# WhatAShot/Electrocardio-Panorama

Measured on AMD Instinct MI355X. Metric: ECG-samples/sec (train step), higher is better.
Workload: dtype f32 (conv products: fp32 operands split into fp16 hi+lo = 22-23 bits, block-scaled, 3 fp16 matrix products each, fp32 accumulate; fp32-class, not IEEE fp32)

## Files before the change

electrocardio_panorama_amd/_lib.py:

```python
import ctypes as C
import os

import torch

_HERE = os.path.dirname(os.path.abspath(__file__))
LIB_PATH = os.path.join(_HERE, "csrc", "libnefnet_hip.so")

NEF_OK = 0
_ERR = {-1: "NEF_E_SHAPE", -2: "NEF_E_NULL", -3: "NEF_E_WORKSPACE", -4: "NEF_E_UNSUPPORTED"}

p = C.c_void_p
i32 = C.c_int
i64 = C.c_int64
f32 = C.c_float
sz = C.c_size_t


class ConvArgs(C.Structure):
    _fields_ = [
        ("x", p), ("wp", p), ("y", p), ("bias", p), ("in_scale", p), ("res", p), ("gate", p), ("mask", p),
        ("x_bs", i64), ("x_gs", i64), ("y_bs", i64), ("y_gs", i64), ("sc_bs", i64), ("sc_gs", i64),
        ("res_bs", i64), ("res_gs", i64), ("gate_bs", i64), ("gate_gs", i64),
        ("B", i32), ("T", i32), ("G", i32), ("Cin_g", i32), ("Cout_g", i32), ("K", i32),
        ("relu", i32), ("gate_scale", f32), ("drop_scale", f32), ("drop_p", f32), ("rng_seed", C.c_uint64),
# ... 116 lines not shown
                ("out_elems", i64), ("signal_elems", i64), ("Bt", i32), ("N", i32), ("A", i32), ("fill", i32), ("dtype", i32),
                ("reserved0", i32)]


class PackDesc(C.Structure):
    _fields_ = [("w", p), ("wp", p), ("G", i32), ("Cog", i32), ("Cig", i32), ("K", i32), ("transpose_flip", i32),
                ("wino", i32), ("src_mode", i32), ("src_Cr", i32)]


SIGNATURES = {
    "nef_abi_version": (i32, []),
    "nef_debug_spin_us": (i32, [f32, i32, p]),
    "nef_stem_fwd": (i32, [p, p, p, i32, i32, i32, p]),
    "nef_stem_bwd_ws_bytes": (sz, [i32]),
    "nef_stem_bwd_weight": (i32, [p, p, p, p, p, sz, i32, i32, i32, p]),
    "nef_pack_weights": (i32, [C.POINTER(PackDesc), i32, p]),
    "nef_pack_bytes": (sz, [C.POINTER(PackDesc)]),
    "nef_live_extent": (i32, [p, p, i32, i32, i32, p]),
    "nef_conv_fwd": (i32, [C.POINTER(ConvArgs), p]),
    "nef_conv_fwd_live": (i32, [C.POINTER(ConvArgs), p, i32, p]),
    "nef_conv_args_bytes": (sz, []),
    "nef_conv_bwd_weight_ws_bytes": (sz, [C.POINTER(BwwArgs)]),
    "nef_conv_bwd_weight": (i32, [C.POINTER(BwwArgs), p]),
    "nef_conv_bwd_weight_live": (i32, [C.POINTER(BwwArgs), p, i32, p]),
    "nef_bww_args_bytes": (sz, []),
    "nef_h2_tail_census_ws_bytes": (sz, [i32, i32, i32]),
    "nef_h2_tail_census": (i32, [p, i64, i64, i32, i32, i32, i32, p, i64, i64, p, p, i32, i32, p, f32, f32, p, sz, p, p, p, p]),
    "nef_bwd_weight_clamp_ends": (i32, [p, p, i64, i64, p, i32, i32, i32, i32, i32, p]),
    "nef_chan_sum_ws_bytes": (sz, [i32]),
    "nef_chan_sum": (i32, [p, p, p, sz, i32, i32, i32, p]),
    "nef_convt2_fwd": (i32, [p, p, p, p, i32, i32, i32, i32, i32, p]),
    "nef_convt2_bwd_data": (i32, [p, p, p, i32, i32, i32, i32, i32, p]),
    "nef_group_transpose": (i32, [p, p, i32, i32, i32, p]),
    "nef_convt2_interleave": (i32, [p, p, p, i32, i32, i32, p]),
    "nef_convt2_deinterleave": (i32, [p, p, i32, i32, i32, p]),
# ... 183 lines not shown
```

electrocardio_panorama_amd/csrc/conv_h2.hip:

```cpp
#include <hip/hip_runtime.h>
#include <stdint.h>
#include <stdlib.h>

#include "nefnet_hip.h"
#include "nef_common.h"


typedef float f32x16 __attribute__((ext_vector_type(16)));
typedef float f32x4 __attribute__((ext_vector_type(4)));
typedef float f32x2 __attribute__((ext_vector_type(2)));
typedef float f32x4_a4 __attribute__((ext_vector_type(4), aligned(4)));
typedef _Float16 h16x8 __attribute__((ext_vector_type(8)));
typedef _Float16 h16x2 __attribute__((ext_vector_type(2)));
typedef unsigned u32x4 __attribute__((ext_vector_type(4)));
typedef unsigned u32x2 __attribute__((ext_vector_type(2)));

namespace {

constexpr int KC = 16;
constexpr int NTO = 256;
constexpr int PRO_MAX_CIN = 512;

__device__ __forceinline__ void split2(float x0, float x1, unsigned& h, unsigned& l) {
    x0 = __builtin_amdgcn_fmed3f(x0, -65000.f, 65000.f);
// ... 77 lines not shown
            const _Float16 h = (_Float16)v;
            const _Float16 l = (_Float16)(v - (float)h);
            const int64_t frag = ((((int64_t)g * nc16 + ci / 16) * K + kk) * ncot + co / 32) * 2;
            const int fl = (co & 31) + 32 * ((ci & 15) >> 3);
            d.wp[(frag * 64 + fl) * 8 + (ci & 7)] = h;
            d.wp[((frag + 1) * 64 + fl) * 8 + (ci & 7)] = l;
        }
    }
}

#define NEF_H2_TRACK1(V) amax_ = fmaxf(amax_, fabsf(V));
#define NEF_H2_TRACK2(V, W) amax_ = fmaxf(amax_, fmaxf(fabsf(V), fabsf(W)));
constexpr int H2_OCC1 = 3;
template <int K, int PRO, int TM, bool PACK = false>
__global__ __launch_bounds__(256, (TM == 1 && (PRO & 2) == 0) ? H2_OCC1 : 2) void conv_h2_kernel(nef_conv_args a_, int tps_, int n_tiles_, int m_tiles_,
                                                                                                const int32_t* live_, int live_add_) {
    constexpr int MT = 64 * TM;
    constexpr bool UP = (PRO & 2) != 0, AFF = (PRO & 1) != 0;
    constexpr bool PH = (PRO & 4) != 0;
    static_assert(!PH || (!UP && K == 3), "phase-stacked input: K = 3, no upsampling prologue");
    constexpr bool PF = (PRO & 8) != 0;
    static_assert(!PF || (!UP && !PH && K == 3 && TM == 2 && !PACK), "polyphase forward: K = 3, 128-row tile");
    constexpr int NS = UP ? 2 : 1;
    constexpr int PAD = (K - 1) / 2;
    constexpr int XROW = NTO + K - 1;
    constexpr int P4 = (XROW + 3) / 4 + 1;
    constexpr int PLANE = 4 * P4 * 32;
    constexpr int HALF = 4 * P4 * 16;
#define NEF_H2_WADDR(R, W) (((W) >> 1) * HALF + (((R) & 3) * P4 + ((R) >> 2)) * 16 + ((W) & 1) * 8)
#define NEF_H2_RPOS(S) ((((S) & 3) * P4 + ((S) >> 2)) * 16)
    constexpr int NIT = (XROW + 63) / 64;
// ... 613 lines not shown
                    sv[k] = keep + __shfl_xor(send, off, 64);
                }
            }
            const int r = lo >> 1;
            const int ch = g * Cog + cobase + (r & 3) + 8 * (r >> 2);
            const int64_t nslot = (int64_t)tps * 2;
            const int64_t slot = (int64_t)b0 * nslot + (int64_t)(t0 / NTO) * 2 + wn;
            if (inb) slot_out[((int64_t)ch * a.B * nslot + slot) * 2 + (lo & 1)] = sv[0];
        }
    }
    return -1.f;
#undef a
    };
    kargs_t* ap_ = (kargs_t*)__builtin_amdgcn_kernarg_segment_ptr();
    (void)a_;
    const float over_ = tile_pass(ap_, (int)blockIdx.x, (int)threadIdx.x, tps_, n_tiles_, m_tiles_, 0.f, false, live_, live_add_);
    if (over_ > 0.f) {
        int e_;
        (void)frexpf(over_, &e_);
        int bid_ = (int)blockIdx.x, tid_ = (int)threadIdx.x, tps2_ = tps_, nt2_ = n_tiles_, mt2_ = m_tiles_;
        asm volatile("" : "+s"(ap_), "+s"(bid_), "+s"(tps2_), "+s"(nt2_), "+s"(mt2_));
        asm volatile("" : "+v"(tid_));
        (void)tile_pass(ap_, bid_, tid_, tps2_, nt2_, mt2_, ldexpf(1.f, 9 - e_ < 100 ? 9 - e_ : 100), true, nullptr, 0);
    }
}

template <int K, int PRO, int TM, bool PACK = false>
int launch_h2(const nef_conv_args& a, hipStream_t st, const int32_t* live = nullptr, int live_add = 0) {
    constexpr int MT = 64 * TM;
    constexpr int XROW = NTO + K - 1;
    constexpr int P4 = (XROW + 3) / 4 + 1;
    constexpr int PLANE = 4 * P4 * 32;
    constexpr size_t lds = (size_t)4 * PLANE + (((PRO & 1) ? 2 * PRO_MAX_CIN : 0) + 8 * MT + 4) * sizeof(float);
    static unsigned long long lds_set = 0;
    if (int e = nef_ensure_dyn_lds(reinterpret_cast<const void*>(&conv_h2_kernel<K, PRO, TM, PACK>), lds, &lds_set)) return e;
    const int tps = PACK ? (NTO + 4) / (a.T + 4) : (a.T + NTO - 1) / NTO;
    const int n_tiles = PACK ? (a.B + tps - 1) / tps : a.B * tps;
    const int m_tiles = a.Cout_g / MT;
    const int64_t blocks = (int64_t)a.G * m_tiles * n_tiles;
    if (blocks <= 0 || blocks > 0x7fffffff) return NEF_E_SHAPE;
    hipLaunchKernelGGL((conv_h2_kernel<K, PRO, TM, PACK>), dim3((unsigned)blocks), dim3(256), lds, st, a, tps, n_tiles, m_tiles, live, live_add);
    return nef_launch_status();
}

}

static bool h2_pack_shape(const nef_conv_args* a) {
    if (!(a->T >= 8 && a->T <= 64 && a->T % 4 == 0 && (a->K == 1 || a->K == 3))) return false;
    const int64_t spt = (NTO + 4) / (a->T + 4);
    const int64_t lim = 0x7fffffff / 4;
    return a->pro_mode == 0 && !a->in_scale && !a->res_scale && !a->gate_rowscale && !a->stats && !a->bnb_slots && spt * a->x_bs < lim && spt * a->y_bs < lim &&
           (!a->res || spt * a->res_bs < lim) && (!a->gate || spt * a->gate_bs < lim);
}

__attribute__((visibility("hidden"))) bool nef_h2_ok(const nef_conv_args* a) {
    return (a->K == 1 || a->K == 3 || a->K == 7) && a->Cout_g % 64 == 0 && a->Cin_g % KC == 0 && a->T % 2 == 0 &&
           (a->T >= NTO / 2 || h2_pack_shape(a)) &&
           ((a->pro_mode >= 0 && a->pro_mode <= 4) || a->pro_mode == 8 || a->pro_mode == 9) && (a->K == 3 || a->pro_mode == 0) &&
           !(a->pro_mode && a->in_scale) &&
           (!a->res_scale || (a->res && !(a->pro_mode & 8))) &&
           ((!a->gate_rowscale && a->stats_mode == 0) || (a->gate && !(a->pro_mode & 8) && (a->stats_mode == 0 || (a->stats_mode == 1 && a->stats && !a->bnb_slots)))) &&
           (!(a->pro_mode & 8) || (a->Cout_g % 128 == 0 && a->T >= NTO / 2 && !a->res && !a->gate && !a->mask && !a->relu && a->drop_p <= 0.f &&
                                   !a->bnb_slots && (int64_t)a->Cout_g * a->T * 4 < 0x7fffffff)) &&
           (a->pro_mode != 4 || (a->T >= NTO / 2 && (int64_t)a->Cin_g * a->T * 4 < 0x7fffffff)) &&
           (!(a->pro_mode & 1) || a->Cin_g <= PRO_MAX_CIN);
}

__attribute__((visibility("hidden"))) int nef_h2_launch(const nef_conv_args* a, hipStream_t st, const int32_t* live, int live_add) {
    if (!nef_h2_ok(a)) return NEF_E_SHAPE;
    if ((a->pro_mode & 1) && !(a->pro_a && a->pro_b && a->pro_Bp > 0)) return NEF_E_NULL;
    const bool wide = a->Cout_g % 128 == 0;
    if (a->T < NTO / 2)
        return a->K == 1 ? launch_h2<1, 0, 1, true>(*a, st) : launch_h2<3, 0, 1, true>(*a, st);
    if (a->K == 7) return wide ? launch_h2<7, 0, 2>(*a, st, live, live_add) : launch_h2<7, 0, 1>(*a, st, live, live_add);
    if (a->K == 1) return wide ? launch_h2<1, 0, 2>(*a, st, live, live_add) : launch_h2<1, 0, 1>(*a, st, live, live_add);
    switch (a->pro_mode) {
        case 0: return wide ? launch_h2<3, 0, 2>(*a, st, live, live_add) : launch_h2<3, 0, 1>(*a, st, live, live_add);
        case 1: return wide ? launch_h2<3, 1, 2>(*a, st) : launch_h2<3, 1, 1>(*a, st);
        case 2: return launch_h2<3, 2, 1>(*a, st);
        case 4: return wide ? launch_h2<3, 4, 2>(*a, st) : launch_h2<3, 4, 1>(*a, st);
        case 8: return launch_h2<3, 8, 2>(*a, st);
        case 9: return launch_h2<3, 9, 2>(*a, st);
        default: return launch_h2<3, 3, 1>(*a, st);
    }
}

__attribute__((visibility("hidden"))) int nef_h2_pack_status(const nef_pack_desc* dp) {
    const nef_pack_desc& d = *dp;
    const int co_n = d.transpose_flip ? d.Cig : d.Cog, ci_n = d.transpose_flip ? d.Cog : d.Cig;
    if (d.G <= 0 || co_n % 32 != 0 || ci_n % 16 != 0 || (d.K != 1 && d.K != 3 && d.K != 7)) return NEF_E_SHAPE;
    if (d.src_mode != 0 && !(d.src_mode == 1 && d.K == 3 && d.Cog % 2 == 0 && d.src_Cr >= 0 &&
                             (d.src_Cr == 0 || (d.src_Cr % 64 == 0 && d.Cog == 2 * d.src_Cr)))) return NEF_E_SHAPE;
// ... 21 lines not shown
```

electrocardio_panorama_amd/csrc/conv_mfma.hip:

```cpp
#include "nef_common.h"
#include <stdlib.h>

typedef float f32x16 __attribute__((ext_vector_type(16)));
typedef float f32x4 __attribute__((ext_vector_type(4)));
typedef float f32x2 __attribute__((ext_vector_type(2)));

#ifndef NEF_MFMA_PART
#define NEF_MFMA_PART 0
#endif
#define NEF_PART(n) (NEF_MFMA_PART == 0 || NEF_MFMA_PART == (n))

namespace {

constexpr int NT = 128;
constexpr int WT = 64;

template <int K> struct StageK;
template <> struct StageK<7> { static constexpr int KC = 16; };
template <int K, int TM> struct FwdStage {
    static constexpr int KC = ((K == 7 || K == 3) && TM == 2) ? 8 : StageK<K>::KC;
};
template <> struct StageK<3> { static constexpr int KC = 16; };
template <> struct StageK<1> { static constexpr int KC = 64; };

// ... 1920 lines not shown
}

__global__ void chan_sum_final(const double* __restrict__ part, float* __restrict__ out, int C, int nsplit) {
    const int c = blockIdx.x * blockDim.x + threadIdx.x;
    if (c >= C) return;
    double s = 0.0;
    for (int sp = 0; sp < nsplit; ++sp) s += part[(int64_t)sp * C + c];
    out[c] = (float)s;
}

constexpr int CHAN_SUM_SPLIT = 16;

}

__attribute__((visibility("hidden"))) bool nef_h2_ok(const nef_conv_args* a);
__attribute__((visibility("hidden"))) int nef_h2_launch(const nef_conv_args* a, hipStream_t st, const int32_t* live, int live_add);
__attribute__((visibility("hidden"))) int nef_h2_pack(const nef_pack_desc* descs, int n, hipStream_t st);
__attribute__((visibility("hidden"))) int nef_h2_pack_status(const nef_pack_desc* d);

__attribute__((visibility("hidden"))) int nef_mfma_wino4_fwd(const nef_conv_args* a, hipStream_t st);
__attribute__((visibility("hidden"))) int nef_mfma_wino_fwd(const nef_conv_args* a, hipStream_t st);

#if NEF_PART(1)
extern "C" {

int nef_abi_version(void) { return 22; }

static int pack_desc_status(const nef_pack_desc& d) {
    NEF_REQUIRE(d.G > 0 && d.Cog > 0 && d.Cig > 0 && d.K > 0 && d.wino >= 0 && d.wino <= 3 &&
                    (!d.wino || d.K == 3 || d.K == 7 || (d.wino == 3 && d.K == 1)), NEF_E_SHAPE);
    NEF_REQUIRE(d.src_mode == 0 || d.wino == 3, NEF_E_UNSUPPORTED);
// ... 43 lines not shown
        for (int i = 0; i < m; ++i) {
            const int64_t e = (int64_t)t.d[i].G * t.d[i].Cog * t.d[i].Cig * (t.d[i].wino ? 1 : t.d[i].K);
            if (e > biggest) biggest = e;
        }
        int gx = (int)nef_cdiv(biggest, 256);
        if (n_f32 == 1) gx = nef_stream_grid(biggest, 256);
        else if (gx > 64) gx = 64;
        hipLaunchKernelGGL(pack_weights_multi_kernel, dim3((unsigned)gx, (unsigned)m), dim3(256), 0, (hipStream_t)stream, t);
    }
    return nef_launch_status();
}

size_t nef_conv_args_bytes(void) { return sizeof(nef_conv_args); }


static int conv_fwd_entry(const nef_conv_args* a, const int32_t* live, int32_t live_add, nef_stream_t stream) {
    NEF_REQUIRE(a && a->x && a->wp && a->y, NEF_E_NULL);
    NEF_REQUIRE(a->B > 0 && a->T > 0 && a->G > 0, NEF_E_SHAPE);
    const int K = a->K;
    NEF_REQUIRE(K == 1 || K == 3 || K == 7, NEF_E_SHAPE);
    NEF_REQUIRE(a->Cout_g % 64 == 0 && a->Cin_g > 0, NEF_E_SHAPE);
    hipStream_t st = (hipStream_t)stream;
    NEF_REQUIRE((!a->stats && !a->bnb_slots) || a->wino == 2 || a->wino == 3, NEF_E_UNSUPPORTED);
    NEF_REQUIRE(!(a->stats && a->bnb_slots), NEF_E_UNSUPPORTED);
    NEF_REQUIRE(!a->bnb_slots || (a->bnb_x && a->bnb_mean && a->bnb_invstd && a->bnb_a && a->bnb_b), NEF_E_NULL);
    NEF_REQUIRE(!a->bnb_slots || a->bnb_Bp > 0, NEF_E_SHAPE);
    NEF_REQUIRE(!a->bnb_slots || !a->bnb_up || a->T % 4 == 0, NEF_E_SHAPE);
    NEF_REQUIRE((!a->res_scale && !a->gate_rowscale && a->stats_mode == 0) || a->wino == 3, NEF_E_UNSUPPORTED);
    if (a->wino == 3) {
        NEF_REQUIRE(nef_h2_ok(a), NEF_E_SHAPE);
        return nef_h2_launch(a, st, live, live_add);
    }
    bool big = (a->Cout_g % 128 == 0);
    if (big) {
        const ColTiling ct0 = make_tiling(a->B, a->T, NT);
        if ((int64_t)a->G * (a->Cout_g / 128) * ct0.n_tiles < 384) big = false;
    }
    const int KC = K == 1 ? FwdStage<1, 1>::KC : (big ? FwdStage<3, 2>::KC : FwdStage<3, 1>::KC);
    static_assert(FwdStage<7, 2>::KC == FwdStage<3, 2>::KC && FwdStage<7, 1>::KC == FwdStage<3, 1>::KC, "stage sizes");
    NEF_REQUIRE(a->Cin_g % KC == 0, NEF_E_SHAPE);
    if (a->wino == 2) return nef_mfma_wino4_fwd(a, st);
    if (a->wino) return nef_mfma_wino_fwd(a, st);
    if (a->pro_mode != 0) {
        NEF_REQUIRE(K == 3 && a->pro_mode >= 1 && a->pro_mode <= 3 && !a->in_scale, NEF_E_UNSUPPORTED);
        NEF_REQUIRE(!(a->pro_mode & 1) || (a->pro_a && a->pro_b && a->pro_Bp > 0), NEF_E_NULL);
        NEF_REQUIRE(!(a->pro_mode & 2) || (a->T % 2 == 0), NEF_E_SHAPE);
// ... 4 lines not shown
        switch (a->pro_mode) {
            case 1: return big ? launch_conv_fwd<3, 2, 1>(*a, st) : launch_conv_fwd<3, 1, 1>(*a, st);
            case 2: return big ? launch_conv_fwd<3, 2, 2>(*a, st) : launch_conv_fwd<3, 1, 2>(*a, st);
            default: return big ? launch_conv_fwd<3, 2, 3>(*a, st) : launch_conv_fwd<3, 1, 3>(*a, st);
        }
    }
    switch (K) {
        case 7: return big ? launch_conv_fwd<7, 2>(*a, st) : launch_conv_fwd<7, 1>(*a, st);
        case 3: return big ? launch_conv_fwd<3, 2>(*a, st) : launch_conv_fwd<3, 1>(*a, st);
        default: return big ? launch_conv_fwd<1, 2>(*a, st) : launch_conv_fwd<1, 1>(*a, st);
    }
}

int nef_conv_fwd(const nef_conv_args* a, nef_stream_t stream) {
    NEF_ENTER();
    return conv_fwd_entry(a, nullptr, 0, stream);
}

int nef_conv_fwd_live(const nef_conv_args* a, const int32_t* live, int32_t live_add, nef_stream_t stream) {
    NEF_ENTER();
    NEF_REQUIRE(live, NEF_E_NULL);
    return conv_fwd_entry(a, live, live_add, stream);
}

int nef_conv_stats_slots(int T, int Cout_g) {
    if (T <= 0 || T % 2 != 0 || Cout_g <= 0 || Cout_g % 64 != 0) return 0;
    const bool wide = (Cout_g % 128 == 0);
    if (T < (wide ? 128 : 256)) return 0;
    const int nto = wide ? 128 : 256;
    return ((T + nto - 1) / nto) * (nto / 128);
}

size_t nef_bww_args_bytes(void) { return sizeof(nef_bww_args); }

size_t nef_conv_bwd_weight_ws_bytes(const nef_bww_args* a) {
    if (!a) return 0;
    const int B = a->B, T = a->T, G = a->G, Cin_g = a->Cin_g, Cout_g = a->Cout_g, K = a->K;
// ... 190 lines not shown
```

electrocardio_panorama_amd/csrc/stem.hip:

```cpp
#include "nef_common.h"

namespace {

constexpr int KW = 15;
constexpr int TP = 64;
constexpr int CPL = 128;

__device__ __forceinline__ void load_window(__amdgpu_buffer_rsrc_t xrow, int L, int tp, float (&xw)[19]) {
    const int base = 4 * tp - 9;
#pragma unroll
    for (int i = 0; i < 19; ++i) {
        const int p = base + i;
        xw[i] = nef_buf_f32(xrow, (p >= 0 && p < L) ? (unsigned)(p * 4) : NEF_OOB, 0);
    }
}

constexpr int FWD_TP = TP - 1;

__global__ __launch_bounds__(256) void stem_fwd_kernel(const float* __restrict__ x, const float* __restrict__ w,
                                                       float* __restrict__ y, int B, int V, int L, int T,
                                                       int tiles_per_row) {
    __shared__ float wl[CPL * 16];
    int bid = blockIdx.x;
    const int tile = bid % tiles_per_row;
// ... 125 lines not shown
    for (int c = 0; c < BW_CPW; ++c)
#pragma unroll
        for (int k = 0; k < KW; ++k) {
            const float s = nef_wave_sum(acc[c][k]);
            if (lane == 0) part[((int64_t)split * V * CPL + ch0 + c) * KW + k] = s;
        }
}

constexpr int MB_SPLIT = 256;
constexpr int MB_HALO = 16;
constexpr int MB_TAIL = 96;
typedef float f32x4s __attribute__((ext_vector_type(4)));

__global__ __launch_bounds__(256) void stem_bwd_weight_mfma_kernel(const float* __restrict__ x, const float* __restrict__ w,
                                                                   const float* __restrict__ gy, float* __restrict__ part,
                                                                   int B, int V, int L, int T) {
    extern __shared__ float xs[];
    const int v = blockIdx.x % V, slot = blockIdx.x / V;
    const int lane = threadIdx.x & 63, wave = __builtin_amdgcn_readfirstlane((int)(threadIdx.x >> 6));
    const int n16 = lane & 15, kk = lane >> 4;
    const int Lc = L / 2;
    const int xlen = MB_HALO + L + MB_TAIL;
    float wb[2][4];
#pragma unroll
    for (int ct = 0; ct < 2; ++ct)
#pragma unroll
        for (int s = 0; s < 4; ++s) {
            const int tap = 4 * s + kk;
            wb[ct][s] = tap < KW ? w[(v * CPL + 32 * wave + 16 * ct + n16) * KW + tap] : 0.f;
        }
    f32x4s acc[2];
#pragma unroll
    for (int ct = 0; ct < 2; ++ct) acc[ct] = f32x4s{0.f, 0.f, 0.f, 0.f};
    for (int b = slot; b < B; b += MB_SPLIT) {
        __syncthreads();
        const float* xrow = x + ((int64_t)b * V + v) * L;
        for (int i = threadIdx.x; i < xlen; i += 256) {
            const int p = i - MB_HALO;
            xs[i] = (p >= 0 && p < L) ? xrow[p] : 0.f;
        }
        __syncthreads();
        const __amdgpu_buffer_rsrc_t grs = nef_rsrc(gy + ((int64_t)b * V * CPL + v * CPL + 32 * wave) * T);
#define NEF_STEM_GLOAD(TP0, DST)                                                                                       \
    _Pragma("unroll") for (int ct_ = 0; ct_ < 2; ++ct_) {                                                           \
        const int tpl_ = (TP0) + 4 * kk;                                                                            \
        DST[ct_] = nef_buf_f32x4(grs, tpl_ + 3 < T ? (unsigned)((n16 * T + tpl_) * 4) : NEF_OOB, (unsigned)(16 * ct_ * T * 4)); \
        if (tpl_ + 3 >= T && tpl_ < T) {                                                                            \
            _Pragma("unroll") for (int r_ = 0; r_ < 4; ++r_)                                                        \
                DST[ct_][r_] = nef_buf_f32(grs, tpl_ + r_ < T ? (unsigned)((n16 * T + tpl_ + r_) * 4) : NEF_OOB,    \
                                           (unsigned)(16 * ct_ * T * 4));                                           \
        }                                                                                                           \
    }
        f32x4s gnext[2];
        NEF_STEM_GLOAD(0, gnext)
        for (int tp0 = 0; tp0 < T; tp0 += 16) {
            f32x4s gcur[2] = {gnext[0], gnext[1]};
            if (tp0 + 16 < T) NEF_STEM_GLOAD(tp0 + 16, gnext)
            const float* p1 = xs + MB_HALO + 4 * (tp0 + n16) - 9 + kk;
            const float* p2 = xs + MB_HALO + 4 * (tp0 + 4 * kk) - 9 + n16;
            float a1[9], a2[9];
#pragma unroll
            for (int o = 0; o < 9; ++o) {
                a1[o] = p1[2 * o];
                a2[o] = p2[2 * o];
            }
#pragma unroll
            for (int ct = 0; ct < 2; ++ct) {
                const int tpl = tp0 + 4 * kk;
                const f32x4s g4 = gcur[ct];
                f32x4s c[3];
#pragma unroll
                for (int i = 0; i < 3; ++i) {
// ... 108 lines not shown
}

int nef_stem_fwd(const float* x, const float* w, float* y, int B, int V, int L, nef_stream_t stream) {
    NEF_ENTER();
    NEF_REQUIRE(x && w && y, NEF_E_NULL);
    NEF_REQUIRE(B > 0 && V > 0 && L >= 4 && L % 4 == 0, NEF_E_SHAPE);
    const int T = L / 4;
    const int tiles = (T + FWD_TP - 1) / FWD_TP;
    hipLaunchKernelGGL(stem_fwd_kernel, dim3((unsigned)((int64_t)B * V * tiles)), dim3(256), 0, (hipStream_t)stream, x,
                       w, y, B, V, L, T, tiles);
    return nef_launch_status();
}

size_t nef_stem_bwd_ws_bytes(int V) { return (size_t)(MB_SPLIT > BW_SPLIT ? MB_SPLIT : BW_SPLIT) * V * CPL * KW * sizeof(float); }

int nef_stem_bwd_weight(const float* x, const float* w, const float* gy, float* gw, void* ws, size_t ws_bytes, int B,
                        int V, int L, nef_stream_t stream) {
    NEF_ENTER();
    NEF_REQUIRE(x && w && gy && gw && ws, NEF_E_NULL);
    NEF_REQUIRE(B > 0 && V > 0 && L >= 4 && L % 4 == 0, NEF_E_SHAPE);
    NEF_REQUIRE(ws_bytes >= nef_stem_bwd_ws_bytes(V), NEF_E_WORKSPACE);
    const int T = L / 4;
    hipStream_t st = (hipStream_t)stream;
    const int n = V * CPL * KW;
    const size_t lds = (size_t)(MB_HALO + L + MB_TAIL) * sizeof(float);
    if (T % 2 == 0 && lds <= 64 * 1024) {
        const int slots = B < MB_SPLIT ? B : MB_SPLIT;
        hipLaunchKernelGGL(stem_bwd_weight_mfma_kernel, dim3((unsigned)(slots * V)), dim3(256), lds, st, x, w, gy, (float*)ws, B,
                           V, L, T);
        hipLaunchKernelGGL(stem_bwd_weight_reduce, dim3((n + 63) / 64), dim3(256), 0, st, (const float*)ws, gw, n, slots);
        return nef_launch_status();
    }
    const int tiles = (T + BW_TP - 1) / BW_TP;
    hipLaunchKernelGGL(stem_bwd_weight_kernel, dim3((unsigned)(BW_SPLIT * V * (CPL / BW_CPB))), dim3(256), 0, st, x, w,
                       gy, (float*)ws, B, V, L, T, tiles);
    hipLaunchKernelGGL(stem_bwd_weight_reduce, dim3((n + 63) / 64), dim3(256), 0, st, (const float*)ws, gw, n, BW_SPLIT);
    return nef_launch_status();
}

}
```

electrocardio_panorama_amd/engine.py:

```python
import os

import torch
from . import _env

from . import ops
from .ops import GV

N_SEG, ROI_BINS = 7, 16
DROP_P = 0.2
BN_EPS, BN_MOM = 1e-5, 0.1


DROPOUT_SITES = ("W_encoder.layer1.0", "W_encoder.layer1.1", "W_encoder.layer1.2", "w_conv.0", "z1_conv.0",
                 "z2_conv1.0", "z2_conv2.0", "z2_conv2.2")


class DropCfg:

    def __init__(self, training, p=DROP_P, masks=None, seed=0, seed_dev=None):
        self.seed_dev = seed_dev
        self.on = bool(training) and p > 0.0
        self.p = p if self.on else 0.0
        self.scale = 1.0 / (1.0 - p) if self.on else 1.0
        self.masks = masks
# ... 25 lines not shown


def block_fwd(xv, P, prefix, K, Cog, drop, in_scale=None, live=None):
    G = xv.G
    h = ops.conv(xv, ops.pack_weight(P[prefix + ".conv1.weight"], G, T=xv.T), Cog, K, relu=True, in_scale=in_scale, live=live,
                 **drop.args(prefix))
    res_conv = (K == 3 and Cog != xv.Cg)
    assert in_scale is None or not res_conv
    if res_conv:
        r = ops.conv(xv, ops.pack_weight(P[prefix + ".residual_conv.weight"], G, T=xv.T), Cog, 1,
                     bias=P[prefix + ".residual_conv.bias"], live=live)
        resv = GV.dense(r, G)
    else:
        resv = xv
    y = ops.conv(GV.dense(h, G), ops.pack_weight(P[prefix + ".conv2.weight"], G, T=xv.T), Cog, K, res=resv, relu=True,
                 res_scale=in_scale, live=_live_add(live, (K - 1) // 2))
    return y, (xv, h, y, prefix, K, Cog, res_conv, drop.scale, in_scale, live)


def block_scale_ok(P, prefix, G, T):
    return all(ops._pack_shape(P[prefix + n], G, False, T, plain=False)[3] == 3 for n in (".conv1.weight", ".conv2.weight")) and T >= 128


def _bwd_f4(K):
    return K in (3, 7)


def _block_pack_requests(P, prefix, G, T, flip):
    w1 = P[prefix + ".conv1.weight"]
    f4 = bool(flip) and _bwd_f4(w1.shape[2])
    reqs = [ops.PackReq(w1, G, flip, T, f4=f4), ops.PackReq(P[prefix + ".conv2.weight"], G, flip, T, f4=f4)]
# ... 52 lines not shown

def _side(device, work=None):
    mode = _env.get("NEF_SIDE_STREAM", "auto")
    if mode == "0" or (mode == "auto" and work is not None and work < _SIDE_MIN_WORK
                       and not torch.cuda.is_current_stream_capturing()):
        return ops._Inline()
    return ops.SideStream.get(device)


def block_bwd(saved, gy, P, grads, out=None, side=None, pre_gated=False, gate_input=False, scale_bwd=False, g2_chan_sum=None):
    xv, h, y, prefix, K, Cog, res_conv, dscale = saved[:8]
    in_scale = saved[8] if len(saved) > 8 else None
    live_x = saved[9] if len(saved) > 9 else None
    live_h = _live_add(live_x, (K - 1) // 2)
    live_y = block_live_out(saved)
    side = side or ops._Inline()
    G, Cig = xv.G, xv.Cg
    g2 = gy if pre_gated else ops.gate(gy, y)
    g2v, hv = GV.dense(g2, G), GV.dense(h, G)
    grads[prefix + ".conv2.weight"] = side.run(lambda: ops.conv_bwd_weight(hv, g2v, K, site=P[prefix + ".conv2.weight"].data_ptr(), live=live_y), h, g2)
    gc1 = ops.conv(g2v, ops.pack_weight(P[prefix + ".conv2.weight"], G, flip=True, T=xv.T, f4=_bwd_f4(K)), Cog, K, gate=hv,
                   gate_scale=dscale, role="conv_bwd_data", live=live_y)
    gc1v = GV.dense(gc1, G)
    grads[prefix + ".conv1.weight"] = side.run(lambda: ops.conv_bwd_weight(xv, gc1v, K, in_scale=in_scale, site=P[prefix + ".conv1.weight"].data_ptr(), live=live_h), xv.t, gc1)
    if res_conv:
        grads[prefix + ".residual_conv.weight"] = side.run(lambda: ops.conv_bwd_weight(xv, g2v, 1, site=P[prefix + ".residual_conv.weight"].data_ptr()), xv.t, g2)
        grads[prefix + ".residual_conv.bias"] = g2_chan_sum if g2_chan_sum is not None else side.run(lambda: ops.chan_sum(g2), g2)
        gres = ops.conv(g2v, ops.pack_weight(P[prefix + ".residual_conv.weight"], G, flip=True, T=xv.T), Cig, 1,
                        role="conv_bwd_data")
        resv = GV.dense(gres, G)
    else:
        resv = g2v
    wp1f = ops.pack_weight(P[prefix + ".conv1.weight"], G, flip=True, T=xv.T, f4=_bwd_f4(K))
    if in_scale is not None and scale_bwd and int(getattr(wp1f, "nef_wino", 0)) == 3 and out is None:
        slots = ops.conv_stats_buffer(wp1f, xv.B, G, Cig, xv.T, xv.t.device)
        if slots is not None:
            gx = ops.conv(gc1v, wp1f, Cig, K, res=resv, gate=xv, gate_scale=1.0, gate_rowscale=in_scale, stats=slots, stats_mode=1,
                          role="conv_bwd_data", live=live_h)
            return gx, ops.slots_to_rows(slots, xv.B)
    return ops.conv(gc1v, wp1f, Cig, K, res=resv,
                    out=out, gate=xv if gate_input else None, gate_scale=1.0, role="conv_bwd_data", live=live_h)


_DEC = (("decoder.1", "0", "1", 128), ("decoder.1", "3", "4", 128), ("decoder.3", "0", "1", 64),
        ("decoder.3", "3", "4", 64))


_HALVES = "decoder.1.double_conv.0.weight#halves"


def _regroup_halves(w, P=None):
    if P is not None:
        hit = P.get(_HALVES)
        if hit is not None and hit[1] is w and hit[2] == w._version:
            return hit[0]
    wg = ops.regroup_halves(w)
# ... 185 lines not shown
            g = ops.conv(gcv, wpf, x.shape[1], 3, role="conv_bwd_data", bnb=bnb)
        g_is_up = bool(up_after and li > 0 and c.shape[2] % 8 == 0 and c.shape[2] >= 16)
        if up_after and li > 0 and not g_is_up:
            g = ops.upsample2_bwd(g)
    return g, bool(saved[0][7]) and not poly_first, shared_B is not None


def _latents(P, x, in_theta, rois, drop, save, pack_side=None):
    B, V, L = x.shape
    T = L // 4
    sv = {}
    r0 = (T - 1) // 2
    win = (r0 - 2, 6) if (T % 2 == 0 and r0 - 2 >= 0 and r0 + 4 <= T) else None
    ops.pack_many(_latent_pack_requests(P, V, T, win, False))
    live = (ops.live_extent(x), 0) if ops.LIVE else None
    a = ops.stem_fwd(x, P["W_encoder.conv1.weight"])
    if pack_side is not None:
        pack_side.join()
    sv["blk_enc"] = []
    for i in range(3):
        a, s = block_fwd(GV.dense(a, V), P, f"W_encoder.layer1.{i}", 7, 128, drop, live=live)
        sv["blk_enc"].append(s)
        live = block_live_out(s)
    e = ops.theta_mlp_fwd(in_theta, P["mlp1.weight"], P["mlp1.bias"])
    if block_scale_ok(P, "w_conv.0", V, T):
        enc, sv["blk_w_conv"] = block_fwd(GV.dense(a, V), P, "w_conv.0", 3, 128, drop, in_scale=(e, V * 128, 128), live=live)
    else:
        ew = ops.chscale_fwd(a, e)
        enc, sv["blk_w_conv"] = block_fwd(GV.dense(ew, V), P, "w_conv.0", 3, 128, drop, live=live)
    live = block_live_out(sv["blk_w_conv"])
# ... 355 lines not shown
    gew = block_bwd(sv["blk_w_conv"], genc, P, grads, side=side, pre_gated=True, scale_bwd=True)
    if isinstance(gew, tuple):
        g, ge = gew
    else:
        g, ge = ops.chscale_bwd(gew, sv["w"], sv["e"], relu_x=True)
    gW1, gb1 = side.run(lambda: ops.theta_mlp_bwd(sv["in_theta"], ge, 128), ge)
    grads["mlp1.weight"], grads["mlp1.bias"] = gW1, gb1
    if early:
        if EARLY_HOOK is not None:
            EARLY_HOOK(P, grads, side)
        else:
            from . import parallel
            parallel.early_reduce(P, grads, getattr(side, "stream", None))
    for i in (2, 1, 0):
        g = block_bwd(sv["blk_enc"][i], g, P, grads, side=side, pre_gated=True, gate_input=(i > 0))
    grads["W_encoder.conv1.weight"] = ops.stem_bwd_weight(sv["x"], P["W_encoder.conv1.weight"], g)


def backward(P, sv, g_outs):
    grads = {}
    side = _side(sv["z1"].device, sv["z1"].numel())
    if "views" in sv:
        gz1, gz2r, gz2b, gz1_sum = _views_bwd(P, sv, g_outs, grads, side)
    else:
        gz1, gz2r, gz2b, gz1_sum = _head_bwd(P, sv, g_outs, grads, side, relu_z1=True)
    _latents_bwd(P, sv, gz1, gz2r, grads, side, z1_pre_gated=True, early=True, gz2b=gz2b, gz1_sum=gz1_sum)
    side.join()
    return grads


def backward2(P, sv, g_outs):
# ... 24 lines not shown
```

electrocardio_panorama_amd/ops.py:

```python
import ctypes as C
import contextlib
import itertools
import os
from typing import NamedTuple, Optional

import torch
from . import _env

from . import _lib

N_SEG, ROI_BINS = 7, 16


def _p(t):
    return None if t is None else t.data_ptr()


def _stream():
    return torch.cuda.current_stream().cuda_stream


def _chk(t, dtype=torch.float32):
    assert t.is_cuda and t.dtype == dtype and t.is_contiguous(), (t.device, t.dtype, t.is_contiguous())
    return t
# ... 152 lines not shown
        _LIVE_ACC_OF[0] = PROFILE
    acc = _LIVE_ACC.setdefault(tag, [0.0, 0])
    acc[0] += frac
    acc[1] += 1
    EXEC_FP16[tag] = 3.0 * acc[0] / acc[1]


def _live_frac(live, pad, T, tile=256):
    if _LIVE_HOST[0] is not live[0]:
        _LIVE_HOST[0], _LIVE_HOST[1] = live[0], live[0].to("cpu", torch.int64)
    tps = (T + tile - 1) // tile
    bound = _LIVE_HOST[1] + int(live[1]) + pad
    return float(((bound + tile - 1) // tile).clamp(0, tps).double().mean()) / tps


def stem_bwd_weight(x, w, gy):
    L = _lib.load()
    _chk(x), _chk(w), _chk(gy)
    B, V, Ln = x.shape
    gw = torch.empty_like(w)
    n = L.nef_stem_bwd_ws_bytes(V)
    ws = workspace(n, x.device)
    ev = _hbm("stem_bwd_weight", x, gy)
    _lib.check(L.nef_stem_bwd_weight(_p(x), _p(w), _p(gy), _p(gw), _p(ws), n, B, V, Ln, _stream()), "nef_stem_bwd_weight")
    _done(ev)
    return gw


_WV = _env.get("NEF_WINOGRAD", "4")
WINOGRAD = _WV != "0"
WINO_FWD = 1 if _WV in ("1", "2") else 2
WINO_BW4 = _WV not in ("1", "2")
WINO_BW7 = _WV not in ("1", "2")


H2 = _env.get("NEF_H2", "1") == "1"


BATCH_HINT = None
# ... 390 lines not shown
                                         _p(invstd), _p(a), _p(b), _p(ws), n, P, N // P, Ct, Ln, eps, momentum, _p(nbt), _stream()),
               "nef_bn_stats_from_slots")
    return mean, invstd, a, b


def _operand(a, xv, in_scale, pro):
    a.x, a.x_bs, a.x_gs = xv.ptr, xv.bs, xv.gs
    if in_scale is not None:
        a.in_scale, a.sc_bs, a.sc_gs = _p(in_scale[0]), in_scale[1], in_scale[2]
    if pro is not None and pro[0]:
        a.pro_mode, a.pro_a, a.pro_b, a.pro_Bp = pro[0], _p(pro[1]), _p(pro[2]), pro[3]


def conv(xv, wp, Cog, K, out=None, bias=None, in_scale=None, res=None, gate=None, gate_scale=1.0, relu=False,
         mask=None, drop_p=0.0, drop_scale=1.0, seed=0, role="conv_fwd", pro=None, seed_dev=None, stats=None, bnb=None,
         x_scale=0.0, tag_extra="", res_scale=None, gate_rowscale=None, stats_mode=0, live=None):
    L = _lib.load()
    if live is not None and not LIVE:
        live = None

    def launch():
        if live is not None:
            _lib.check(L.nef_conv_fwd_live(C.byref(a), _p(live[0]), int(live[1]), _stream()), "nef_conv_fwd_live")
        else:
            _lib.check(L.nef_conv_fwd(C.byref(a), _stream()), "nef_conv_fwd")
    T_out = xv.T * 2 if (pro is not None and pro[0] & 2) else xv.T
    if out is None:
        y = torch.empty(xv.B, xv.G * Cog, T_out, device=xv.t.device, dtype=torch.float32)
        out = GV.dense(y, xv.G)
    a = _lib.ConvArgs()
    _operand(a, xv, in_scale, pro)
    a.wp, a.y, a.y_bs, a.y_gs = _p(wp), out.ptr, out.bs, out.gs
    a.bias = _p(bias)
    a.res = res.ptr if res is not None else None
    a.gate = gate.ptr if gate is not None else None
    a.mask = _p(mask)
    if res is not None:
# ... 1755 lines not shown
```

include/nefnet_hip.h:

```cpp
#ifndef NEFNET_HIP_H
#define NEFNET_HIP_H

#include <stddef.h>
#include <stdint.h>

#ifdef __cplusplus
extern "C" {
#endif

#define NEF_OK 0
#define NEF_E_SHAPE (-1)
#define NEF_E_NULL (-2)
#define NEF_E_WORKSPACE (-3)
#define NEF_E_UNSUPPORTED (-4)

#define NEF_N_SEG 7
#define NEF_ROI_BINS 16

typedef void* nef_stream_t;

int nef_abi_version(void);

int nef_debug_spin_us(float us, int wgs, nef_stream_t stream);

int nef_stem_fwd(const float* x, const float* w, float* y, int B, int V, int L, nef_stream_t stream);
int nef_live_extent(const float* x, int32_t* live, int B, int V, int L, nef_stream_t stream);
size_t nef_stem_bwd_ws_bytes(int V);
int nef_stem_bwd_weight(const float* x, const float* w, const float* gy, float* gw, void* ws, size_t ws_bytes,
                        int B, int V, int L, nef_stream_t stream);

typedef struct nef_pack_desc {
    const float* w;
    float* wp;
    int32_t G, Cog, Cig, K, transpose_flip, wino;
    int32_t src_mode, src_Cr;
} nef_pack_desc;
size_t nef_pack_bytes(const nef_pack_desc* d);
int nef_pack_weights(const nef_pack_desc* descs, int n, nef_stream_t stream);

typedef struct nef_conv_args {
    const float* x;
    const float* wp;
    float* y;
    const float* bias;
// ... 26 lines not shown
    float x_scale;
    int32_t reserved0;
    const float* x_amax;
    float* x_amax_next;
    int32_t* x_clamped;
    const float* res_scale;
    int64_t rs_bs, rs_gs;
    const float* gate_rowscale;
    int64_t gr_bs, gr_gs;
    int32_t stats_mode;
    int32_t reserved1;
} nef_conv_args;

int nef_conv_fwd(const nef_conv_args* a, nef_stream_t stream);
int nef_conv_fwd_live(const nef_conv_args* a, const int32_t* live, int32_t live_add, nef_stream_t stream);
size_t nef_conv_args_bytes(void);

typedef struct nef_bww_args {
    const float* x;
    const float* gy;
    float* gw;
    void* ws;
    const float* in_scale;
    const float* pro_a;
    const float* pro_b;
    const float* x_amax;
    const float* gy_amax;
    float* x_amax_next;
    float* gy_amax_next;
    int32_t* clamped;
// ... 556 lines not shown
```

Before: 9816.

## Zero-fill dead conv tiles early and clip stem weight-grad to live extent

In the h2 conv kernel, tiles lying fully beyond the per-sample live extent (and beyond the residual's live extent when a residual is added) now write zeros directly and exit, skipping the MFMA work. This applies only when there is no bias, stats or BN slots. A new residual-aware live entry point carries the residual's extent through the encoder block forward and backward-data calls. The stem backward-weight kernel also receives the live extent and stops its time loop at the live end rounded up to 16, which assumes gradients and inputs past that point contribute nothing.

Result: faster. 10070, median of 6 (+2.6%).

```diff
diff --git a/electrocardio_panorama_amd/_lib.py b/electrocardio_panorama_amd/_lib.py
--- a/electrocardio_panorama_amd/_lib.py
+++ b/electrocardio_panorama_amd/_lib.py
@@ -154,11 +154,13 @@
     "nef_stem_fwd": (i32, [p, p, p, i32, i32, i32, p]),
     "nef_stem_bwd_ws_bytes": (sz, [i32]),
     "nef_stem_bwd_weight": (i32, [p, p, p, p, p, sz, i32, i32, i32, p]),
+    "nef_stem_bwd_weight_live": (i32, [p, p, p, p, p, sz, i32, i32, i32, p, p]),
     "nef_pack_weights": (i32, [C.POINTER(PackDesc), i32, p]),
     "nef_pack_bytes": (sz, [C.POINTER(PackDesc)]),
     "nef_live_extent": (i32, [p, p, i32, i32, i32, p]),
     "nef_conv_fwd": (i32, [C.POINTER(ConvArgs), p]),
     "nef_conv_fwd_live": (i32, [C.POINTER(ConvArgs), p, i32, p]),
+    "nef_conv_fwd_live_res": (i32, [C.POINTER(ConvArgs), p, i32, i32, p]),
     "nef_conv_args_bytes": (sz, []),
     "nef_conv_bwd_weight_ws_bytes": (sz, [C.POINTER(BwwArgs)]),
     "nef_conv_bwd_weight": (i32, [C.POINTER(BwwArgs), p]),
diff --git a/electrocardio_panorama_amd/csrc/conv_h2.hip b/electrocardio_panorama_amd/csrc/conv_h2.hip
--- a/electrocardio_panorama_amd/csrc/conv_h2.hip
+++ b/electrocardio_panorama_amd/csrc/conv_h2.hip
@@ -115,7 +115,7 @@
 constexpr int H2_OCC1 = 3;
 template <int K, int PRO, int TM, bool PACK = false>
 __global__ __launch_bounds__(256, (TM == 1 && (PRO & 2) == 0) ? H2_OCC1 : 2) void conv_h2_kernel(nef_conv_args a_, int tps_, int n_tiles_, int m_tiles_,
-                                                                                                const int32_t* live_, int live_add_) {
+                                                                                                const int32_t* live_, int live_add_, int zf_, int res_add_) {
     constexpr int MT = 64 * TM;
     constexpr bool UP = (PRO & 2) != 0, AFF = (PRO & 1) != 0;
     constexpr bool PH = (PRO & 4) != 0;
@@ -759,6 +759,37 @@
     };
     kargs_t* ap_ = (kargs_t*)__builtin_amdgcn_kernarg_segment_ptr();
     (void)a_;
+    if constexpr (PRO == 0 && !PACK) {
+        if (zf_) {
+            const int tile = (int)blockIdx.x % n_tiles_, gm = (int)blockIdx.x / n_tiles_;
+            const int mt = gm % m_tiles_, g = gm / m_tiles_;
+            const int full = (n_tiles_ / (8 * tps_)) * (8 * tps_);
+            int b0, t0;
+            if (tile < full) {
+                const int grp = tile / (8 * tps_), r = tile % (8 * tps_);
+                b0 = grp * 8 + (r & 7);
+                t0 = (r >> 3) * NTO;
+            } else {
+                b0 = tile / tps_;
+                t0 = (tile - b0 * tps_) * NTO;
+            }
+            const int e = live_[b0 * ap_->G + g];
+            const bool dead = t0 - PAD >= e + live_add_;
+            if (dead && (zf_ == 1 || t0 >= e + res_add_)) {
+                const int T = ap_->T;
+                const int t = t0 + 4 * ((int)threadIdx.x & 63);
+                float* const yp = ap_->y + (int64_t)b0 * ap_->y_bs + (int64_t)g * ap_->y_gs + (int64_t)(mt * MT) * T + t;
+                if (t + 3 < T) {
+#pragma unroll 8
+                    for (int r = (int)threadIdx.x >> 6; r < MT; r += 4) *reinterpret_cast<f32x4_a4*>(yp + (int64_t)r * T) = f32x4_a4{0.f, 0.f, 0.f, 0.f};
+                } else if (t < T) {
+#pragma unroll 8
+                    for (int r = (int)threadIdx.x >> 6; r < MT; r += 4) *reinterpret_cast<f32x2*>(yp + (int64_t)r * T) = f32x2{0.f, 0.f};
+                }
+                return;
+            }
+        }
+    }
     const float over_ = tile_pass(ap_, (int)blockIdx.x, (int)threadIdx.x, tps_, n_tiles_, m_tiles_, 0.f, false, live_, live_add_);
     if (over_ > 0.f) {
         int e_;
@@ -771,7 +802,7 @@
 }
 
 template <int K, int PRO, int TM, bool PACK = false>
-int launch_h2(const nef_conv_args& a, hipStream_t st, const int32_t* live = nullptr, int live_add = 0) {
+int launch_h2(const nef_conv_args& a, hipStream_t st, const int32_t* live = nullptr, int live_add = 0, const int* res_add = nullptr) {
     constexpr int MT = 64 * TM;
     constexpr int XROW = NTO + K - 1;
     constexpr int P4 = (XROW + 3) / 4 + 1;
@@ -784,7 +815,10 @@
     const int m_tiles = a.Cout_g / MT;
     const int64_t blocks = (int64_t)a.G * m_tiles * n_tiles;
     if (blocks <= 0 || blocks > 0x7fffffff) return NEF_E_SHAPE;
-    hipLaunchKernelGGL((conv_h2_kernel<K, PRO, TM, PACK>), dim3((unsigned)blocks), dim3(256), lds, st, a, tps, n_tiles, m_tiles, live, live_add);
+    int zf = 0;
+    if (PRO == 0 && !PACK && live && !a.bias && !a.stats && !a.bnb_slots) zf = !a.res ? 1 : (res_add ? 2 : 0);
+    hipLaunchKernelGGL((conv_h2_kernel<K, PRO, TM, PACK>), dim3((unsigned)blocks), dim3(256), lds, st, a, tps, n_tiles, m_tiles, live, live_add, zf,
+                       res_add ? *res_add : 0);
     return nef_launch_status();
 }
 
@@ -811,16 +845,16 @@
            (!(a->pro_mode & 1) || a->Cin_g <= PRO_MAX_CIN);
 }
 
-__attribute__((visibility("hidden"))) int nef_h2_launch(const nef_conv_args* a, hipStream_t st, const int32_t* live, int live_add) {
+__attribute__((visibility("hidden"))) int nef_h2_launch(const nef_conv_args* a, hipStream_t st, const int32_t* live, int live_add, const int* res_add) {
     if (!nef_h2_ok(a)) return NEF_E_SHAPE;
     if ((a->pro_mode & 1) && !(a->pro_a && a->pro_b && a->pro_Bp > 0)) return NEF_E_NULL;
     const bool wide = a->Cout_g % 128 == 0;
     if (a->T < NTO / 2)
         return a->K == 1 ? launch_h2<1, 0, 1, true>(*a, st) : launch_h2<3, 0, 1, true>(*a, st);
-    if (a->K == 7) return wide ? launch_h2<7, 0, 2>(*a, st, live, live_add) : launch_h2<7, 0, 1>(*a, st, live, live_add);
-    if (a->K == 1) return wide ? launch_h2<1, 0, 2>(*a, st, live, live_add) : launch_h2<1, 0, 1>(*a, st, live, live_add);
+    if (a->K == 7) return wide ? launch_h2<7, 0, 2>(*a, st, live, live_add, res_add) : launch_h2<7, 0, 1>(*a, st, live, live_add, res_add);
+    if (a->K == 1) return wide ? launch_h2<1, 0, 2>(*a, st, live, live_add, res_add) : launch_h2<1, 0, 1>(*a, st, live, live_add, res_add);
     switch (a->pro_mode) {
-        case 0: return wide ? launch_h2<3, 0, 2>(*a, st, live, live_add) : launch_h2<3, 0, 1>(*a, st, live, live_add);
+        case 0: return wide ? launch_h2<3, 0, 2>(*a, st, live, live_add, res_add) : launch_h2<3, 0, 1>(*a, st, live, live_add, res_add);
         case 1: return wide ? launch_h2<3, 1, 2>(*a, st) : launch_h2<3, 1, 1>(*a, st);
         case 2: return launch_h2<3, 2, 1>(*a, st);
         case 4: return wide ? launch_h2<3, 4, 2>(*a, st) : launch_h2<3, 4, 1>(*a, st);
diff --git a/electrocardio_panorama_amd/csrc/conv_mfma.hip b/electrocardio_panorama_amd/csrc/conv_mfma.hip
--- a/electrocardio_panorama_amd/csrc/conv_mfma.hip
+++ b/electrocardio_panorama_amd/csrc/conv_mfma.hip
@@ -1958,7 +1958,7 @@
 }
 
 __attribute__((visibility("hidden"))) bool nef_h2_ok(const nef_conv_args* a);
-__attribute__((visibility("hidden"))) int nef_h2_launch(const nef_conv_args* a, hipStream_t st, const int32_t* live, int live_add);
+__attribute__((visibility("hidden"))) int nef_h2_launch(const nef_conv_args* a, hipStream_t st, const int32_t* live, int live_add, const int* res_add);
 __attribute__((visibility("hidden"))) int nef_h2_pack(const nef_pack_desc* descs, int n, hipStream_t st);
 __attribute__((visibility("hidden"))) int nef_h2_pack_status(const nef_pack_desc* d);
 
@@ -2032,7 +2032,7 @@
 size_t nef_conv_args_bytes(void) { return sizeof(nef_conv_args); }
 
 
-static int conv_fwd_entry(const nef_conv_args* a, const int32_t* live, int32_t live_add, nef_stream_t stream) {
+static int conv_fwd_entry(const nef_conv_args* a, const int32_t* live, int32_t live_add, const int32_t* res_add, nef_stream_t stream) {
     NEF_REQUIRE(a && a->x && a->wp && a->y, NEF_E_NULL);
     NEF_REQUIRE(a->B > 0 && a->T > 0 && a->G > 0, NEF_E_SHAPE);
     const int K = a->K;
@@ -2047,7 +2047,7 @@
     NEF_REQUIRE((!a->res_scale && !a->gate_rowscale && a->stats_mode == 0) || a->wino == 3, NEF_E_UNSUPPORTED);
     if (a->wino == 3) {
         NEF_REQUIRE(nef_h2_ok(a), NEF_E_SHAPE);
-        return nef_h2_launch(a, st, live, live_add);
+        return nef_h2_launch(a, st, live, live_add, res_add);
     }
     bool big = (a->Cout_g % 128 == 0);
     if (big) {
@@ -2082,13 +2082,19 @@
 
 int nef_conv_fwd(const nef_conv_args* a, nef_stream_t stream) {
     NEF_ENTER();
-    return conv_fwd_entry(a, nullptr, 0, stream);
+    return conv_fwd_entry(a, nullptr, 0, nullptr, stream);
 }
 
 int nef_conv_fwd_live(const nef_conv_args* a, const int32_t* live, int32_t live_add, nef_stream_t stream) {
     NEF_ENTER();
     NEF_REQUIRE(live, NEF_E_NULL);
-    return conv_fwd_entry(a, live, live_add, stream);
+    return conv_fwd_entry(a, live, live_add, nullptr, stream);
+}
+
+int nef_conv_fwd_live_res(const nef_conv_args* a, const int32_t* live, int32_t live_add, int32_t res_add, nef_stream_t stream) {
+    NEF_ENTER();
+    NEF_REQUIRE(live && a && a->res, NEF_E_NULL);
+    return conv_fwd_entry(a, live, live_add, &res_add, stream);
 }
 
 int nef_conv_stats_slots(int T, int Cout_g) {
diff --git a/electrocardio_panorama_amd/csrc/stem.hip b/electrocardio_panorama_amd/csrc/stem.hip
--- a/electrocardio_panorama_amd/csrc/stem.hip
+++ b/electrocardio_panorama_amd/csrc/stem.hip
@@ -163,13 +163,13 @@
 
 __global__ __launch_bounds__(256) void stem_bwd_weight_mfma_kernel(const float* __restrict__ x, const float* __restrict__ w,
                                                                    const float* __restrict__ gy, float* __restrict__ part,
-                                                                   int B, int V, int L, int T) {
+                                                                   int B, int V, int L, int T, const int32_t* __restrict__ live) {
     extern __shared__ float xs[];
     const int v = blockIdx.x % V, slot = blockIdx.x / V;
     const int lane = threadIdx.x & 63, wave = __builtin_amdgcn_readfirstlane((int)(threadIdx.x >> 6));
     const int n16 = lane & 15, kk = lane >> 4;
     const int Lc = L / 2;
-    const int xlen = MB_HALO + L + MB_TAIL;
+    const int xlen_full = MB_HALO + L + MB_TAIL;
     float wb[2][4];
 #pragma unroll
     for (int ct = 0; ct < 2; ++ct)
@@ -183,6 +183,12 @@
     for (int ct = 0; ct < 2; ++ct) acc[ct] = f32x4s{0.f, 0.f, 0.f, 0.f};
     for (int b = slot; b < B; b += MB_SPLIT) {
         __syncthreads();
+        int Tb = T, xlen = xlen_full;
+        if (live) {
+            const int e = live[b * V + v];
+            const int e16 = (e + 15) & ~15;
+            if (e16 < T) Tb = e16 > 0 ? e16 : 0, xlen = MB_HALO + 4 * Tb + 8;
+        }
         const float* xrow = x + ((int64_t)b * V + v) * L;
         for (int i = threadIdx.x; i < xlen; i += 256) {
             const int p = i - MB_HALO;
@@ -202,9 +208,9 @@
     }
         f32x4s gnext[2];
         NEF_STEM_GLOAD(0, gnext)
-        for (int tp0 = 0; tp0 < T; tp0 += 16) {
+        for (int tp0 = 0; tp0 < Tb; tp0 += 16) {
             f32x4s gcur[2] = {gnext[0], gnext[1]};
-            if (tp0 + 16 < T) NEF_STEM_GLOAD(tp0 + 16, gnext)
+            if (tp0 + 16 < Tb) NEF_STEM_GLOAD(tp0 + 16, gnext)
             const float* p1 = xs + MB_HALO + 4 * (tp0 + n16) - 9 + kk;
             const float* p2 = xs + MB_HALO + 4 * (tp0 + 4 * kk) - 9 + n16;
             float a1[9], a2[9];
@@ -343,9 +349,8 @@
 
 size_t nef_stem_bwd_ws_bytes(int V) { return (size_t)(MB_SPLIT > BW_SPLIT ? MB_SPLIT : BW_SPLIT) * V * CPL * KW * sizeof(float); }
 
-int nef_stem_bwd_weight(const float* x, const float* w, const float* gy, float* gw, void* ws, size_t ws_bytes, int B,
-                        int V, int L, nef_stream_t stream) {
-    NEF_ENTER();
+static int stem_bwd_weight_entry(const float* x, const float* w, const float* gy, float* gw, void* ws, size_t ws_bytes, int B,
+                                 int V, int L, const int32_t* live, nef_stream_t stream) {
     NEF_REQUIRE(x && w && gy && gw && ws, NEF_E_NULL);
     NEF_REQUIRE(B > 0 && V > 0 && L >= 4 && L % 4 == 0, NEF_E_SHAPE);
     NEF_REQUIRE(ws_bytes >= nef_stem_bwd_ws_bytes(V), NEF_E_WORKSPACE);
@@ -356,7 +361,7 @@
     if (T % 2 == 0 && lds <= 64 * 1024) {
         const int slots = B < MB_SPLIT ? B : MB_SPLIT;
         hipLaunchKernelGGL(stem_bwd_weight_mfma_kernel, dim3((unsigned)(slots * V)), dim3(256), lds, st, x, w, gy, (float*)ws, B,
-                           V, L, T);
+                           V, L, T, live);
         hipLaunchKernelGGL(stem_bwd_weight_reduce, dim3((n + 63) / 64), dim3(256), 0, st, (const float*)ws, gw, n, slots);
         return nef_launch_status();
     }
@@ -367,4 +372,17 @@
     return nef_launch_status();
 }
 
-}
+int nef_stem_bwd_weight(const float* x, const float* w, const float* gy, float* gw, void* ws, size_t ws_bytes, int B,
+                        int V, int L, nef_stream_t stream) {
+    NEF_ENTER();
+    return stem_bwd_weight_entry(x, w, gy, gw, ws, ws_bytes, B, V, L, nullptr, stream);
+}
+
+int nef_stem_bwd_weight_live(const float* x, const float* w, const float* gy, float* gw, void* ws, size_t ws_bytes, int B,
+                             int V, int L, const int32_t* live, nef_stream_t stream) {
+    NEF_ENTER();
+    NEF_REQUIRE(live, NEF_E_NULL);
+    return stem_bwd_weight_entry(x, w, gy, gw, ws, ws_bytes, B, V, L, live, stream);
+}
+
+}
diff --git a/electrocardio_panorama_amd/engine.py b/electrocardio_panorama_amd/engine.py
--- a/electrocardio_panorama_amd/engine.py
+++ b/electrocardio_panorama_amd/engine.py
@@ -63,7 +63,7 @@
     else:
         resv = xv
     y = ops.conv(GV.dense(h, G), ops.pack_weight(P[prefix + ".conv2.weight"], G, T=xv.T), Cog, K, res=resv, relu=True,
-                 res_scale=in_scale, live=_live_add(live, (K - 1) // 2))
+                 res_scale=in_scale, live=_live_add(live, (K - 1) // 2), res_live=None if (res_conv or live is None) else live[1])
     return y, (xv, h, y, prefix, K, Cog, res_conv, drop.scale, in_scale, live)
 
 
@@ -146,6 +146,7 @@
     live_x = saved[9] if len(saved) > 9 else None
     live_h = _live_add(live_x, (K - 1) // 2)
     live_y = block_live_out(saved)
+    res_live = None if (res_conv or live_y is None) else live_y[1]
     side = side or ops._Inline()
     G, Cig = xv.G, xv.Cg
     g2 = gy if pre_gated else ops.gate(gy, y)
@@ -168,10 +169,10 @@
         slots = ops.conv_stats_buffer(wp1f, xv.B, G, Cig, xv.T, xv.t.device)
         if slots is not None:
             gx = ops.conv(gc1v, wp1f, Cig, K, res=resv, gate=xv, gate_scale=1.0, gate_rowscale=in_scale, stats=slots, stats_mode=1,
-                          role="conv_bwd_data", live=live_h)
+                          role="conv_bwd_data", live=live_h, res_live=res_live)
             return gx, ops.slots_to_rows(slots, xv.B)
     return ops.conv(gc1v, wp1f, Cig, K, res=resv,
-                    out=out, gate=xv if gate_input else None, gate_scale=1.0, role="conv_bwd_data", live=live_h)
+                    out=out, gate=xv if gate_input else None, gate_scale=1.0, role="conv_bwd_data", live=live_h, res_live=res_live)
 
 
 _DEC = (("decoder.1", "0", "1", 128), ("decoder.1", "3", "4", 128), ("decoder.3", "0", "1", 64),
@@ -387,6 +388,7 @@
     win = (r0 - 2, 6) if (T % 2 == 0 and r0 - 2 >= 0 and r0 + 4 <= T) else None
     ops.pack_many(_latent_pack_requests(P, V, T, win, False))
     live = (ops.live_extent(x), 0) if ops.LIVE else None
+    sv["stem_live"] = live[0] if live is not None else None
     a = ops.stem_fwd(x, P["W_encoder.conv1.weight"])
     if pack_side is not None:
         pack_side.join()
@@ -772,7 +774,7 @@
             parallel.early_reduce(P, grads, getattr(side, "stream", None))
     for i in (2, 1, 0):
         g = block_bwd(sv["blk_enc"][i], g, P, grads, side=side, pre_gated=True, gate_input=(i > 0))
-    grads["W_encoder.conv1.weight"] = ops.stem_bwd_weight(sv["x"], P["W_encoder.conv1.weight"], g)
+    grads["W_encoder.conv1.weight"] = ops.stem_bwd_weight(sv["x"], P["W_encoder.conv1.weight"], g, live=sv.get("stem_live"))
 
 
 def backward(P, sv, g_outs):
diff --git a/electrocardio_panorama_amd/ops.py b/electrocardio_panorama_amd/ops.py
--- a/electrocardio_panorama_amd/ops.py
+++ b/electrocardio_panorama_amd/ops.py
@@ -190,7 +190,7 @@
     return float(((bound + tile - 1) // tile).clamp(0, tps).double().mean()) / tps
 
 
-def stem_bwd_weight(x, w, gy):
+def stem_bwd_weight(x, w, gy, live=None):
     L = _lib.load()
     _chk(x), _chk(w), _chk(gy)
     B, V, Ln = x.shape
@@ -198,7 +198,11 @@
     n = L.nef_stem_bwd_ws_bytes(V)
     ws = workspace(n, x.device)
     ev = _hbm("stem_bwd_weight", x, gy)
-    _lib.check(L.nef_stem_bwd_weight(_p(x), _p(w), _p(gy), _p(gw), _p(ws), n, B, V, Ln, _stream()), "nef_stem_bwd_weight")
+    if live is not None and LIVE and LIVE_WGRAD:
+        assert live.shape == (B, V) and live.dtype == torch.int32
+        _lib.check(L.nef_stem_bwd_weight_live(_p(x), _p(w), _p(gy), _p(gw), _p(ws), n, B, V, Ln, _p(live), _stream()), "nef_stem_bwd_weight_live")
+    else:
+        _lib.check(L.nef_stem_bwd_weight(_p(x), _p(w), _p(gy), _p(gw), _p(ws), n, B, V, Ln, _stream()), "nef_stem_bwd_weight")
     _done(ev)
     return gw
 
@@ -619,13 +623,15 @@
 
 def conv(xv, wp, Cog, K, out=None, bias=None, in_scale=None, res=None, gate=None, gate_scale=1.0, relu=False,
          mask=None, drop_p=0.0, drop_scale=1.0, seed=0, role="conv_fwd", pro=None, seed_dev=None, stats=None, bnb=None,
-         x_scale=0.0, tag_extra="", res_scale=None, gate_rowscale=None, stats_mode=0, live=None):
+         x_scale=0.0, tag_extra="", res_scale=None, gate_rowscale=None, stats_mode=0, live=None, res_live=None):
     L = _lib.load()
     if live is not None and not LIVE:
         live = None
 
     def launch():
-        if live is not None:
+        if live is not None and res is not None and res_live is not None:
+            _lib.check(L.nef_conv_fwd_live_res(C.byref(a), _p(live[0]), int(live[1]), int(res_live), _stream()), "nef_conv_fwd_live_res")
+        elif live is not None:
             _lib.check(L.nef_conv_fwd_live(C.byref(a), _p(live[0]), int(live[1]), _stream()), "nef_conv_fwd_live")
         else:
             _lib.check(L.nef_conv_fwd(C.byref(a), _stream()), "nef_conv_fwd")
diff --git a/include/nefnet_hip.h b/include/nefnet_hip.h
--- a/include/nefnet_hip.h
+++ b/include/nefnet_hip.h
@@ -28,6 +28,8 @@
 size_t nef_stem_bwd_ws_bytes(int V);
 int nef_stem_bwd_weight(const float* x, const float* w, const float* gy, float* gw, void* ws, size_t ws_bytes,
                         int B, int V, int L, nef_stream_t stream);
+int nef_stem_bwd_weight_live(const float* x, const float* w, const float* gy, float* gw, void* ws, size_t ws_bytes,
+                             int B, int V, int L, const int32_t* live, nef_stream_t stream);
 
 typedef struct nef_pack_desc {
     const float* w;
@@ -84,6 +86,7 @@
 
 int nef_conv_fwd(const nef_conv_args* a, nef_stream_t stream);
 int nef_conv_fwd_live(const nef_conv_args* a, const int32_t* live, int32_t live_add, nef_stream_t stream);
+int nef_conv_fwd_live_res(const nef_conv_args* a, const int32_t* live, int32_t live_add, int32_t res_add, nef_stream_t stream);
 size_t nef_conv_args_bytes(void);
 
 typedef struct nef_bww_args {
```
